# NDLOHGRP/pyReCoDe

Measured on AMD Instinct MI355X. Metric: frames/sec + GB/s in, 4096x4096 uint16 @1% sparsity, 1/2/4/8 GPU, higher is better.
Workload: dtype u16; 1 GPU; 4096x4096 uint16, 1.00% sparsity, L1 + LZ4 frame, source_bit_depth 16, batch 64 frames/GPU/step, 256-frame stack/GPU in HBM; parallelism=dp1 (contiguous frame blocks per rank; single process: no collective), gather_every=0, gathers_issued_in_all=0, launch=single process, collective_ranks=1

## Files before the change

### pyrecode_amd/csrc/rc_api.hip

```cpp
#include "rc_host.h"

thread_local std::string g_last_error;
WorkerPool *g_pool = new WorkerPool;
Util g_utils[RC_MAX_DEV];
thread_local Util *t_util = nullptr;


struct rc_ctx {
    int device = 0;
    hipStream_t own_stream = nullptr, stream = nullptr;
    uint32_t nx = 0, ny = 0, depth = 0, level = 0, op_mode = 0, scheme = 0, clevel = 0, max_batch = 0;
    uint32_t emit = rc::EMIT_RAW;
    rc::Scratch sc, sets[2];
    int cur = 0;
    int last = 0;
    hipStream_t pstream = nullptr;
    hipStream_t pstream_b = nullptr;
    hipStream_t last_ps = nullptr;
    bool two_chains = false;
    hipEvent_t ev_red[2] = {}, ev_post[2] = {}, ev_in[2] = {};
    bool post_pending[2] = {false, false};
    bool pipelined = false;
    bool thr_set = false;
    bool keep_bitmap = true;
    uint32_t src_bytes = 2;
    uint32_t *thr32 = nullptr;
    uint32_t last_n = 0;
    uint8_t *d_frames = nullptr;  uint64_t d_frames_cap = 0;
    uint8_t *d_out = nullptr;     uint64_t d_out_cap = 0;
    uint8_t *d_dark = nullptr;    uint64_t d_dark_cap = 0;
    uint64_t *d_rec_off = nullptr;
    uint32_t *d_md = nullptr;
    void *d_ztab = nullptr;
    bool modelled = false, model_ready = false;
    rc::ZstdModel *d_model = nullptr, *h_model = nullptr;
    rc::ZstdSample *d_sample = nullptr, *h_sample = nullptr;
    uint32_t l2_sum = 0;
    rc::u32x2 *d_l2_node[2] = {};
    uint16_t *d_l2_base[2] = {};
    rc::BatchStatus *h_status = nullptr;
    rc::BatchStatus *d_first_err = nullptr;
    uint32_t batch_seq = 0;
    const uint8_t *prev_out = nullptr, *prev_rec = nullptr, *prev_md = nullptr;
    uint64_t prev_out_cap = 0;
    uint32_t prev_n = 0;
    hipEvent_t ev[5] = {};
// ... 87 lines not shown
        sc.pixraw_stride = ((sc.N * 2 + 15) & ~15ull) + 32;
        sc.nchunk_max = (uint32_t)((sc.N * 2 + PIX_CHUNK - 1) / PIX_CHUNK) + 1;
        HIP_TRY(hipMalloc((void **)&sc.pixraw, B * sc.pixraw_stride + 64));
        HIP_TRY(hipMalloc((void **)&sc.pix_chunks, B * (uint64_t)sc.nchunk_max * PIX_SLOT + 64));
        HIP_TRY(hipMalloc((void **)&sc.chunk_size, B * (uint64_t)sc.nchunk_max * 4));
        HIP_TRY(hipMalloc((void **)&sc.chunk_off, B * (uint64_t)sc.nchunk_max * 4));
        HIP_TRY(hipMalloc((void **)&sc.frame_pbytes, B * 4));
        HIP_TRY(hipMemset(sc.frame_pbytes, 0, B * 4));
    }
    HIP_TRY(hipMemset(sc.frame_nnz, 0, B * 4));
    HIP_TRY(hipMemset(sc.frame_cbytes, 0, B * 4));
    HIP_TRY(hipMemset(sc.status, 0, sizeof(BatchStatus)));
    return RC_OK;
}

static int ctx_alloc(rc_ctx *c)
{
    using namespace rc;
    const uint64_t B = c->max_batch;
    RC_ON_DEVICE(c->device);
    HIP_TRY(hipStreamCreateWithFlags(&c->own_stream, hipStreamNonBlocking));
    HIP_TRY(hipStreamCreateWithFlags(&c->pstream, hipStreamNonBlocking));
    {
        int lo = 0, hi = 0;
        HIP_TRY(hipDeviceGetStreamPriorityRange(&lo, &hi));
        HIP_TRY(hipStreamCreateWithPriority(&c->pstream_b, hipStreamNonBlocking, hi));
    }
    c->last_ps = c->pstream;
    c->stream = c->own_stream;
    HIP_TRY(hipMalloc((void **)&c->sc.thr, c->sc.N * 2));
    HIP_TRY(hipMalloc((void **)&c->d_first_err, sizeof(BatchStatus)));
    HIP_TRY(hipMemset(c->d_first_err, 0, sizeof(BatchStatus)));
    c->sc.first_err = c->d_first_err;
    for (Scratch &set : c->sets) {
        set = c->sc;
        int r = alloc_set(c, set);
        if (r != RC_OK) return r;
    }
    c->two_chains = false;
    if (c->level == 2) {
        const uint64_t ids = (uint64_t)c->sc.ntiles * rc::TILE_PX;
        HIP_TRY(hipMalloc((void **)&c->d_l2_node[0], B * ids * 8));
        HIP_TRY(hipMemset(c->d_l2_node[0], 0, B * ids * 8));
        HIP_TRY(hipMalloc((void **)&c->d_l2_base[0], B * (uint64_t)c->sc.ntiles * 64 * 2));
        for (int i = 0; i < 2; ++i) {
            Scratch &set = c->sets[i];
            set.l2_node = c->d_l2_node[0]; set.l2_ids_per_frame = ids; set.l2_base = c->d_l2_base[0];
        }
    }
    c->sc = c->sets[0];
    if (c->emit == EMIT_ZSTD) {
        std::vector<uint8_t> tab(zstd_tables_bytes());
        zstd_tables_host(tab.data());
        HIP_TRY(hipMalloc(&c->d_ztab, tab.size()));
        HIP_TRY(hipMemcpy(c->d_ztab, tab.data(), tab.size(), hipMemcpyHostToDevice));
        c->modelled = c->clevel != 0;
        if (c->modelled) {
            HIP_TRY(hipMalloc((void **)&c->d_model, sizeof(ZstdModel)));
            HIP_TRY(hipMalloc((void **)&c->d_sample, sizeof(ZstdSample)));
            HIP_TRY(hipHostMalloc((void **)&c->h_model, sizeof(ZstdModel), hipHostMallocDefault));
            HIP_TRY(hipHostMalloc((void **)&c->h_sample, sizeof(ZstdSample), hipHostMallocDefault));
        }
    }
    HIP_TRY(hipMalloc((void **)&c->d_rec_off, (B + 1) * 8));
    HIP_TRY(hipMalloc((void **)&c->d_md, B * 3 * 4));
    HIP_TRY(hipHostMalloc((void **)&c->h_status, 2 * sizeof(BatchStatus), hipHostMallocDefault));
// ... 27 lines not shown
        *status = fail(RC_ERR_UNSUPPORTED, "reduction_level 4 (centroiding) is not implemented on device");
        return nullptr;
    }
    if (reduction_level == 2 && nx > 65535u) {
        *status = fail(RC_ERR_UNSUPPORTED, "reduction_level 2 needs nx <= 65535");
        return nullptr;
    }
    if (src_bit_depth < 1 || src_bit_depth > 32) {
        *status = fail(RC_ERR_UNSUPPORTED, "source_bit_depth must be 1..32 (uint8 / uint16 / uint32 source frames)");
        return nullptr;
    }
    int ndev = 0;
    if (hipGetDeviceCount(&ndev) != hipSuccess || device_id < 0 || device_id >= ndev) {
        (void)hipGetLastError();
        *status = fail(RC_ERR_DEVICE, "no such HIP device (this library has no CPU path)");
        return nullptr;
    }
    rc_ctx *c = new (std::nothrow) rc_ctx();
    if (!c) {
        *status = fail(RC_ERR_DEVICE, "out of host memory");
        return nullptr;
    }
    c->device = device_id;
    c->nx = nx; c->ny = ny; c->depth = src_bit_depth; c->level = reduction_level; c->op_mode = op_mode;
    c->scheme = scheme; c->clevel = clevel; c->max_batch = max_batch;
    c->emit = (op_mode == 1 && rc_scheme_on_device(scheme)) ? scheme : rc::EMIT_RAW;
    rc::Scratch &sc = c->sc;
    sc.N = (uint64_t)nx * ny;
    sc.ntiles = (uint32_t)((sc.N + rc::TILE_PX - 1) / rc::TILE_PX);
    sc.nb = (sc.N + 7) / 8;
    sc.nb_stride = (uint64_t)sc.ntiles * rc::TILE_BM;
    sc.max_batch = max_batch;
    sc.guarded_loads = getenv("RC_REDUCE_GUARDED_LOADS") != nullptr;
    int rcode = ctx_alloc(c);
    if (rcode != RC_OK) {
        *status = rcode;
        std::string keep = g_last_error;
        rc_ctx_destroy(c);
        g_last_error = keep;
        return nullptr;
    }
    return c;
}

RC_EXPORT int rc_ctx_destroy(rc_ctx *c)
{
    if (!c) return RC_OK;
    DeviceGuard dev_guard_;
    (void)dev_guard_.enter(c->device);
    if (c->stream) (void)hipStreamSynchronize(c->stream);
    if (c->pstream) (void)hipStreamSynchronize(c->pstream);
    if (c->pstream_b) (void)hipStreamSynchronize(c->pstream_b);
    if (c->own_stream) (void)hipStreamSynchronize(c->own_stream);
    for (rc::Scratch &sc : c->sets) {
        void *per_set[] = {sc.bitmap, sc.pix_slots, sc.tile_cnt, sc.tile_off, sc.tile_next, sc.blk_slots, sc.blk_size, sc.blk_aux, sc.zl_acc,
                           sc.blk_off, sc.frame_nnz, sc.frame_cbytes, sc.scan_part, sc.status, sc.pixraw, sc.pix_chunks, sc.chunk_size, 
                           sc.chunk_off, sc.frame_pbytes};
        for (void *b : per_set)
            if (b) (void)hipFree(b);
    }
    for (auto &p : c->pipe) {
        void *dev[] = {p.d_in, p.d_out, p.d_rec, p.d_md, p.d_val};
        for (void *b : dev) if (b) (void)hipFree(b);
        void *host[] = {p.h_rec, p.h_md, p.h_stat, p.h_val};
        for (void *b : host) if (b) (void)hipHostFree(b);
        hipEvent_t evs[] = {p.ev_h2d, p.ev_done, p.ev_fetch, p.ev_val};
        for (hipEvent_t e : evs) if (e) (void)hipEventDestroy(e);
    }
    if (c->copy_stream) { (void)hipStreamSynchronize(c->copy_stream); (void)hipStreamDestroy(c->copy_stream); }
    if (c->d2h_stream) { (void)hipStreamSynchronize(c->d2h_stream); (void)hipStreamDestroy(c->d2h_stream); }
    if (c->h_model) (void)hipHostFree(c->h_model);
    if (c->h_sample) (void)hipHostFree(c->h_sample);
    void *bufs[] = {c->sc.thr, c->thr32, c->d_first_err, c->d_frames, c->d_out, c->d_dark, c->d_rec_off,
                    c->d_md, c->d_ztab, c->d_model, c->d_sample, c->d_l2_node[0], c->d_l2_node[1], c->d_l2_base[0], c->d_l2_base[1]};
    for (void *b : bufs)
        if (b) (void)hipFree(b);
    hipEvent_t sync_ev[] = {c->ev_red[0], c->ev_red[1], c->ev_post[0], c->ev_post[1], c->ev_in[0], c->ev_in[1]};
    for (hipEvent_t e : sync_ev)
        if (e) (void)hipEventDestroy(e);
    if (c->pstream) (void)hipStreamDestroy(c->pstream);
    if (c->pstream_b) (void)hipStreamDestroy(c->pstream_b);
    if (c->h_status) (void)hipHostFree(c->h_status);
    for (auto &e : c->ev)
        if (e) (void)hipEventDestroy(e);
    for (auto &e : c->prof_ev) (void)hipEventDestroy(e);
    if (c->own_stream) (void)hipStreamDestroy(c->own_stream);
    delete c;
    return RC_OK;
}

RC_EXPORT int rc_ctx_set_stream(rc_ctx *c, void *hip_stream)
{
    if (!c) return fail(RC_ERR_BAD_ARG, "ctx is NULL");
    c->stream = hip_stream ? reinterpret_cast<hipStream_t>(hip_stream) : c->own_stream;
    return RC_OK;
}

RC_EXPORT int rc_set_threshold(rc_ctx *c, const void *thr)
{
    if (!c || !thr) return fail(RC_ERR_BAD_ARG, "ctx / thr is NULL");
    if (c->depth > 16 && c->src_bytes != 4) return fail(RC_ERR_BAD_ARG, "src_bit_depth > 16 means uint32 sources: rc_ctx_set_source_bytes(ctx, 4) first");
    RC_ON_DEVICE(c->device);
    HIP_TRY(hipMemcpyAsync(c->src_bytes == 4 ? (void *)c->thr32 : (void *)c->sc.thr, thr, c->sc.N * (c->src_bytes == 4 ? 4 : 2),
                           is_device_ptr(thr) ? hipMemcpyDeviceToDevice : hipMemcpyHostToDevice,
                           c->stream));
    HIP_TRY(hipStreamSynchronize(c->stream));
// ... 710 lines not shown
```

### pyrecode_amd/csrc/rc_launch.h

```cpp
#pragma once
#include <hip/hip_runtime.h>
#include <stdint.h>

#include "../../include/recode_hip.h"
#include "rc_device.h"

namespace rc {

constexpr uint32_t COMB_OFF = 0u;
constexpr uint32_t COMB_BEHIND_BLOCK = 1u;
constexpr uint32_t COMB_AT_BLK_SLOT = 2u;

struct Scratch {
    uint64_t N = 0;
    uint32_t ntiles = 0;
    uint64_t nb = 0;
    uint64_t nb_stride = 0;
    uint32_t max_batch = 0;
    bool guarded_loads = false;
    uint16_t *thr = nullptr;
    uint8_t *bitmap = nullptr;
    uint16_t *pix_slots = nullptr;
    uint32_t pix_slot_bytes = SLOT_PX * 2;
    uint32_t *tile_cnt = nullptr;
    uint32_t *tile_off = nullptr;
    uint32_t *tile_next = nullptr;
    uint8_t *blk_slots = nullptr;
    uint32_t blk_stride = BLK_SLOT;
    uint32_t comb = COMB_OFF;
    uint32_t *blk_size = nullptr;
    uint32_t *blk_aux = nullptr;
    uint32_t *zl_acc = nullptr;
    uint32_t *blk_off = nullptr;
    uint32_t *frame_nnz = nullptr;
    uint32_t *frame_cbytes = nullptr;
    uint32_t *scan_part = nullptr;
    BatchStatus *status = nullptr;
    BatchStatus *first_err = nullptr;
    uint8_t *pixraw = nullptr;
    uint64_t pixraw_stride = 0;
    uint8_t *pix_chunks = nullptr;
    uint32_t *chunk_size = nullptr;
    uint32_t *chunk_off = nullptr;
    uint32_t *frame_pbytes = nullptr;
    uint32_t nchunk_max = 0;
    const void *zm_model = nullptr;
    const void *zm_lit_code = nullptr;
    uint32_t zm_valid = 0, zm_budget = 0, zm_seq_bits = 12;
    u32x2 *l2_node = nullptr;
    uint64_t l2_ids_per_frame = 0;
    uint16_t *l2_base = nullptr;
};

// ... 86 lines not shown
```

### pyrecode_amd/csrc/rc_reduce.hip

```cpp
#include <cstddef>
#include <cstdlib>
#include <type_traits>

#include "rc_launch.h"
#include "rc_record.h"
#include "rc_pack.h"
#ifdef RC_PHASE_TIMING
__device__ unsigned long long g_phase[16];
#define RC_LZ4_PHASE 1
#endif
#include "rc_lz4_block.h"
#include "rc_zstd_wave.h"
#include "rc_deflate_block.h"

namespace rc {

#ifdef RC_PHASE_TIMING
#define RC_PHASE_BEGIN unsigned long long ph_t_ = __builtin_amdgcn_s_memtime(); unsigned long long ph_a_[8] = {};
#define RC_PHASE(i) do { const unsigned long long ph_n_ = __builtin_amdgcn_s_memtime(); ph_a_[i] = ph_n_ - ph_t_; ph_t_ = ph_n_; \
        if ((i) == 6 && lane_id() == 0 && (blockIdx.x & 63u) == 0) { for (int q_ = 0; q_ < 7; ++q_) atomicAdd(&g_phase[q_], ph_a_[q_]); atomicAdd(&g_phase[7], 1ull); } } while (0)
#else
#define RC_PHASE_BEGIN
#define RC_PHASE(i) do { } while (0)
#endif
constexpr int REDUCE_BZ = 4;

__device__ __forceinline__ uint32_t pk_sub_sat_u16(uint32_t a, uint32_t b)
{
    uint32_t r;
    asm("v_pk_sub_u16 %0, %1, %2 clamp" : "=v"(r) : "v"(a), "v"(b));
    return r;
}
__device__ __forceinline__ uint32_t pk_add_u16(uint32_t a, uint32_t b)
{
    uint32_t r;
    asm("v_pk_add_u16 %0, %1, %2" : "=v"(r) : "v"(a), "v"(b));
    return r;
}
__device__ __forceinline__ uint32_t pk_min_u16(uint32_t a, uint32_t b)
{
    uint32_t r;
    asm("v_pk_min_u16 %0, %1, %2" : "=v"(r) : "v"(a), "v"(b));
    return r;
}

__global__ void k_threshold(const uint16_t *__restrict__ dark, uint32_t eps16, uint64_t N, uint16_t *__restrict__ thr)
{
    uint64_t i = (uint64_t)blockIdx.x * blockDim.x + threadIdx.x;
    const uint64_t stride = (uint64_t)gridDim.x * blockDim.x;
    for (; i < N; i += stride) thr[i] = (uint16_t)(dark[i] + eps16);
}

__global__ void k_threshold8(const uint8_t *__restrict__ dark, uint32_t eps8, uint64_t N, uint16_t *__restrict__ thr)
{
    uint64_t i = (uint64_t)blockIdx.x * blockDim.x + threadIdx.x;
    const uint64_t stride = (uint64_t)gridDim.x * blockDim.x;
// ... 98 lines not shown
    default: asm volatile("global_load_dwordx4 %0, %1, off offset:3072 nt" : "=&v"(xr) : "v"(p) : "memory"); break;
    }
}
__device__ __forceinline__ void vm_issue_load1(u32x2 &xr, const uint8_t *p, int r)
{
    switch (r) {
    case 0: asm volatile("global_load_dwordx2 %0, %1, off nt" : "=&v"(xr) : "v"(p) : "memory"); break;
    case 1: asm volatile("global_load_dwordx2 %0, %1, off offset:512 nt" : "=&v"(xr) : "v"(p) : "memory"); break;
    case 2: asm volatile("global_load_dwordx2 %0, %1, off offset:1024 nt" : "=&v"(xr) : "v"(p) : "memory"); break;
    case 3: asm volatile("global_load_dwordx2 %0, %1, off offset:1536 nt" : "=&v"(xr) : "v"(p) : "memory"); break;
    case 4: asm volatile("global_load_dwordx2 %0, %1, off offset:2048 nt" : "=&v"(xr) : "v"(p) : "memory"); break;
    case 5: asm volatile("global_load_dwordx2 %0, %1, off offset:2560 nt" : "=&v"(xr) : "v"(p) : "memory"); break;
    case 6: asm volatile("global_load_dwordx2 %0, %1, off offset:3072 nt" : "=&v"(xr) : "v"(p) : "memory"); break;
    default: asm volatile("global_load_dwordx2 %0, %1, off offset:3584 nt" : "=&v"(xr) : "v"(p) : "memory"); break;
    }
}
template <class X>
__device__ __forceinline__ void vm_wait_loads(uint32_t later, X (&x)[R])
{
    switch (later) {
    case 1: asm volatile("s_waitcnt vmcnt(1)" ::: "memory"); break;
    case 2: asm volatile("s_waitcnt vmcnt(2)" ::: "memory"); break;
    case 3: asm volatile("s_waitcnt vmcnt(3)" ::: "memory"); break;
    case 4: asm volatile("s_waitcnt vmcnt(4)" ::: "memory"); break;
    case 5: asm volatile("s_waitcnt vmcnt(5)" ::: "memory"); break;
    case 6: asm volatile("s_waitcnt vmcnt(6)" ::: "memory"); break;
    case 7: asm volatile("s_waitcnt vmcnt(7)" ::: "memory"); break;
    case 8: asm volatile("s_waitcnt vmcnt(8)" ::: "memory"); break;
    default: asm volatile("s_waitcnt vmcnt(0)" ::: "memory"); break;
    }
    asm volatile("" : "+v"(x[0]), "+v"(x[1]), "+v"(x[2]), "+v"(x[3]), "+v"(x[4]), "+v"(x[5]), "+v"(x[6]), "+v"(x[7]) :: "memory");
}

constexpr int STAGE_CAP = 256;
struct __attribute__((aligned(16))) WaveStage {
    uint16_t val[TILE_PX];
    uint16_t out[STAGE_CAP];
};
static_assert(offsetof(WaveStage, out) == sizeof(uint16_t) * TILE_PX && STAGE_CAP >= 64, "compact_dense_in_place: `out` lies right behind `val`, an entry per lane");

__device__ __forceinline__ uint32_t store_lines2(const uint8_t *s0, uint8_t *d0, uint32_t q0, const uint8_t *s1, uint8_t *d1, uint32_t q1)
{
    const uint32_t total = q0 + q1, lane = (uint32_t)lane_id();
    for (uint32_t base = 0; base < total; base += 64) {
        const uint32_t i = base + lane;
        if (i < total) {
            const bool second = i >= q0;
            const uint32_t j = second ? i - q0 : i;
            const u32x4 v = *reinterpret_cast<const u32x4 *>((second ? s1 : s0) + 16 * j);
            *reinterpret_cast<u32x4 *>((second ? d1 : d0) + 16 * j) = v;
        }
    }
    return (total + 63u) >> 6;
}

template <bool LEVEL1, int CODEC, bool KEEP_BITMAP>
__device__ __forceinline__ uint32_t flush_pending(const Pending &p, uint32_t tile, uint32_t n_blk, uint8_t *__restrict__ bitmap,
                                                  uint64_t nb_stride, uint16_t *__restrict__ pix_slots, uint32_t *__restrict__ tile_cnt,
                                                  uint8_t *__restrict__ blk_slots, uint32_t *__restrict__ blk_size, Lz4Lds *lz,
                                                  const WaveStage *st, uint32_t blk_stride, uint32_t comb, uint32_t *__restrict__ blk_aux)
{
    if (!p.valid) return 0;
    const int lane = lane_id();
    uint32_t nst = 0;
    const uint8_t *s0 = nullptr, *s1 = nullptr;
    uint8_t *d0 = nullptr, *d1 = nullptr;
// ... 84 lines not shown
{
    const int lane = lane_id();
    uint32_t *out32 = reinterpret_cast<uint32_t *>(st->out);
    *reinterpret_cast<u32x2 *>(out32 + 2 * lane) = u32x2{0u, 0u};
    __builtin_amdgcn_wave_barrier();
    const uint16_t *mine = st->val + 64 * lane;
    uint64_t q = (uint64_t)own[0] | ((uint64_t)own[1] << 32);
    uint32_t left = cnt, P = 12u * exc;
    do {
        uint32_t x[4];
#pragma unroll
        for (int k = 0; k < 4; ++k) {
            const uint32_t i = q ? (uint32_t)__builtin_ctzll(q) : 0u;
            q &= q - 1;
            x[k] = mine[i];
        }
#pragma unroll
        for (int k = 0; k < 4; ++k) x[k] = (uint32_t)k < left ? (x[k] & 0xFFFu) : 0u;
        const uint32_t lo = x[0] | (x[1] << 12) | (x[2] << 24), hi = (x[2] >> 8) | (x[3] << 4);
        const uint32_t w = P >> 5, sh = P & 31u;
        const uint64_t a = (uint64_t)lo << sh, b = (uint64_t)hi << sh;
        const uint32_t d0 = (uint32_t)a, d1 = (uint32_t)(a >> 32) | (uint32_t)b, d2 = (uint32_t)(b >> 32);
        if (left) {
            __hip_atomic_fetch_or(&out32[w], d0, __ATOMIC_RELAXED, __HIP_MEMORY_SCOPE_WAVEFRONT);
            if (d1) __hip_atomic_fetch_or(&out32[w + 1], d1, __ATOMIC_RELAXED, __HIP_MEMORY_SCOPE_WAVEFRONT);
            if (d2) __hip_atomic_fetch_or(&out32[w + 2], d2, __ATOMIC_RELAXED, __HIP_MEMORY_SCOPE_WAVEFRONT);
        }
        left = left > 4u ? left - 4u : 0u;
        P += 48u;
    } while (__builtin_amdgcn_ballot_w64(left != 0) != 0);
    __builtin_amdgcn_wave_barrier();
}

template <bool ALIGNED, bool ASMLOAD, bool LEVEL1, int CODEC, bool KEEP_BITMAP, bool RAWVAL, int SB>
__device__ __forceinline__ void reduce_one_frame(typename Src<SB>::X (&x)[R], const typename Src<SB>::T *__restrict__ cur, const typename Src<SB>::T *__restrict__ next, bool have_next,
                                                 const u32x4 (&t)[R], uint64_t lane_px0, uint64_t N, bool full,
                                                 uint32_t f, uint32_t tile, uint64_t ft, uint32_t n_blk, uint8_t *__restrict__ bitmap,
                                                 uint64_t nb_stride, uint16_t *__restrict__ pix_slots,
                                                 uint32_t *__restrict__ tile_cnt, uint8_t *__restrict__ blk_slots,
                                                 uint32_t *__restrict__ blk_size, Lz4Lds *s_lz, uint8_t *s_bm, WaveStage *st,
                                                 Pending &pend, uint32_t &stores_behind, const ZmParams &zp, uint32_t blk_stride, uint32_t comb,
                                                 uint32_t *__restrict__ blk_aux)
{
    const int lane = lane_id();
    RC_PHASE_BEGIN
    if (ASMLOAD) vm_wait_loads(stores_behind, x);
    else if (ALIGNED && full) {
        typedef typename Src<SB>::X XU __attribute__((aligned(SB)));
        const XU *p = reinterpret_cast<const XU *>(cur + lane_px0);
#pragma unroll
        for (int r = 0; r < R; ++r) x[r] = __builtin_nontemporal_load(p + r * (GROUP_PX / 8));
    } else {
#pragma unroll
        for (int r = 0; r < R; ++r) x[r] = load8<ALIGNED, true, SB>(cur, lane_px0 + (uint64_t)r * GROUP_PX, N, 0);
    }
    RC_PHASE(0);
    uint32_t m8[R];
#pragma unroll
    for (int r = 0; r < R; ++r) {
        const u32x4 tt = t[r];
        u32x4 xv = widen8(x[r]);
#pragma unroll
        for (int k = 0; k < 4; ++k) xv[k] = pk_sub_sat_u16(xv[k], tt[k]);
        const uint32_t one = 0x00010001u;
        uint32_t M = 0;
#pragma unroll
        for (int k = 3; k >= 0; --k)
            M = __builtin_amdgcn_udot2(__builtin_bit_cast(u16x2, pk_min_u16(xv[k], one)),
                                       __builtin_bit_cast(u16x2, (uint32_t)((1u << (2 * k)) | (2u << (2 * k + 16)))), M, false);
        m8[r] = M;
        if (LEVEL1) {
            u32x4 v = xv;
            if (RAWVAL) {
#pragma unroll
                for (int k = 0; k < 4; ++k) v[k] = pk_add_u16(v[k], tt[k]);
            }
            (reinterpret_cast<u32x4 *>(st->val) + lane)[r * 64] = v;
        }
        if (ASMLOAD && have_next) vm_issue_load1(x[r], next + lane_px0, r);
    }
    RC_PHASE(1);
    RC_PHASE(2);
    pend.valid = true;
    pend.ft = ft;
    pend.f = f;
    pend.cnt = 0;
    pend.csize = 0;
    pend.buf = st->out;
    if (LEVEL1 || KEEP_BITMAP || CODEC) {
        uint8_t *bm = CODEC ? s_lz->raw : s_bm;
#pragma unroll
        for (int r = 0; r < R; ++r) bm[r * 64 + lane] = (uint8_t)m8[r];
        __builtin_amdgcn_wave_barrier();
        pend.own = *reinterpret_cast<const u32x2 *>(&bm[lane * 8]);
    }
    RC_PHASE(3);
    if (LEVEL1) {
        const uint32_t cnt = (uint32_t)__builtin_popcount(pend.own[0]) + (uint32_t)__builtin_popcount(pend.own[1]);
        const uint32_t inc = wave_incl_scan(cnt);
        const uint32_t wave_total = wave_last(inc);
        bool packed = false;
        if (pend.depth == 12 && wave_total <= FUSED12_CAP) {
            if (wave_total) compact_pack12(st, pend.own, inc - cnt, cnt);
            packed = true;
        } else if (wave_total <= (uint32_t)STAGE_CAP) {
#pragma unroll
            for (int h = 0; h < 2; ++h) {
                const uint16_t *mine = st->val + 64 * lane + 32 * h;
                uint32_t qh = pend.own[h];
                uint32_t o = inc - cnt + (h ? (uint32_t)__builtin_popcount(pend.own[0]) : 0u);
                while (qh) {
                    const uint32_t i0 = (uint32_t)__builtin_ctz(qh);
// ... 19 lines not shown
    RC_PHASE(4);
    if (CODEC == CODEC_LZ4_RUNS) {
        const uint64_t bytes = (uint64_t)pend.own[0] | ((uint64_t)pend.own[1] << 32);
        pend.csize = lz4_encode_block<false>(bytes, n_blk, *s_lz);
    }
    if (CODEC == CODEC_LZ4_EVENTS) {
        const uint64_t bytes = (uint64_t)pend.own[0] | ((uint64_t)pend.own[1] << 32);
        pend.csize = lz4_encode_block<true>(bytes, n_blk, *s_lz);
    }
    if (CODEC == CODEC_ZSTD_FAST) {
        const uint64_t bytes = (uint64_t)pend.own[0] | ((uint64_t)pend.own[1] << 32);
        pend.csize = zstd_tokenize_block(bytes, n_blk, pend.last, *s_lz, pend.staged);
    }
    if (CODEC == CODEC_ZSTD_MODELLED) {
        const uint64_t bytes = (uint64_t)pend.own[0] | ((uint64_t)pend.own[1] << 32);
        pend.csize = zstd_tokenize_block_m(bytes, n_blk, pend.last, *s_lz, pend.staged, zp);
    }
    if (CODEC == CODEC_DEFLATE) {
        const uint64_t bytes = (uint64_t)pend.own[0] | ((uint64_t)pend.own[1] << 32);
        pend.aux = deflate_adler_word(bytes, tile);
        pend.csize = deflate_encode_block<true>(bytes, n_blk, pend.last, *s_lz);
    }
    if (CODEC == CODEC_BLOSC) {
        const uint64_t bytes = (uint64_t)pend.own[0] | ((uint64_t)pend.own[1] << 32);
        pend.cown = bitshuffle_block(bytes, n_blk, *s_lz);
        pend.csize = lz4_encode_block(pend.cown, n_blk, *s_lz);
    }
    RC_PHASE(5);
    stores_behind = flush_pending<LEVEL1, CODEC, KEEP_BITMAP>(pend, tile, n_blk, bitmap, nb_stride, pix_slots, tile_cnt, blk_slots, blk_size, s_lz, st, blk_stride, comb, blk_aux);
    pend.valid = false;
    RC_PHASE(6);
}

template <int RWAVES, int BZ, bool ALIGNED, bool ASMLOAD, bool LEVEL1, int CODEC, bool KEEP_BITMAP, bool RAWVAL, int SB>
__global__ __launch_bounds__(64 * RWAVES) __attribute__((amdgpu_waves_per_eu((ALIGNED && ASMLOAD) ? ((RWAVES == 4 && LEVEL1) ? 3 : 4) : 1))) void k_reduce_tiles(const typename Src<SB>::T *__restrict__ frames,
                                                       const uint16_t *__restrict__ thr, uint64_t N, uint32_t ntiles,
                                                       uint32_t tile0, uint32_t tile_end,
                                                       uint32_t B, uint32_t ngroups, uint64_t nb,
                                                       uint8_t *__restrict__ bitmap, uint64_t nb_stride,
                                                       uint16_t *__restrict__ pix_slots, uint32_t *__restrict__ tile_cnt,
                                                       uint8_t *__restrict__ blk_slots, uint32_t *__restrict__ blk_size, uint32_t depth,
                                                       BatchStatus *__restrict__ status, ZmParams zm, uint32_t blk_stride, uint32_t comb,
                                                       uint32_t *__restrict__ blk_aux)
{
    if (blockIdx.x == 0 && threadIdx.x == 0) { status->code = 0; status->frame = 0; status->total = 0; }
    __shared__ uint16_t s_code[CODEC == CODEC_ZSTD_MODELLED ? 256 : 2];
    if (CODEC == CODEC_ZSTD_MODELLED) {
        for (uint32_t i = threadIdx.x; i < 128; i += 64 * RWAVES) reinterpret_cast<uint32_t *>(s_code)[i] = reinterpret_cast<const uint32_t *>(zm.lit_code)[i];
        __syncthreads();
        zm.lit_code = s_code;
    }
    __shared__ Lz4Lds s_lz[CODEC ? RWAVES : 1];
    __shared__ __attribute__((aligned(16))) uint8_t s_bm[CODEC ? 1 : RWAVES][CODEC ? 16 : TILE_BM];
    __shared__ WaveStage s_stage[LEVEL1 ? RWAVES : 1];

    const uint32_t xcd = blockIdx.x & 7u, j = blockIdx.x >> 3;
    const uint32_t grp = j % ngroups;
    const uint32_t tblock = (j / ngroups) * 8u + xcd;
    const int lane = lane_id();
    const int w = __builtin_amdgcn_readfirstlane((int)(threadIdx.x >> 6));
    const uint32_t tile = tile0 + tblock * RWAVES + w;
    if (tile >= tile_end) return;
    const uint64_t lane_px0 = (uint64_t)tile * TILE_PX + (uint64_t)lane * 8;
    const uint32_t f0 = grp * BZ;
    if (f0 >= B) return;
    const bool full = (uint64_t)(tile + 1) * TILE_PX <= N;

    typename Src<SB>::X xa[R];
    if (ASMLOAD) vm_issue_loads(xa, frames + (uint64_t)f0 * N + lane_px0);
    u32x4 t[R];
#pragma unroll
    for (int r = 0; r < R; ++r) t[r] = load8<ALIGNED, false, 2>(thr, lane_px0 + (uint64_t)r * GROUP_PX, N, 0xFFFF);
    const uint32_t n_blk = (uint32_t)min((uint64_t)TILE_BM, nb - (uint64_t)tile * TILE_BM);
    Lz4Lds *lz = &s_lz[CODEC ? w : 0];
    uint8_t *bm = s_bm[CODEC ? 0 : w];
    WaveStage *st = &s_stage[LEVEL1 ? w : 0];
    Pending pend;
    pend.valid = false;
    pend.ft = 0; pend.f = 0; pend.cnt = 0; pend.csize = 0; pend.own = u32x2{0u, 0u};
    pend.staged = 0; pend.last = tile + 1 == ntiles; pend.cown = 0; pend.aux = 0;
    pend.depth = (LEVEL1 && !RAWVAL) ? depth : 16u;
    pend.buf = nullptr;

    uint32_t stores_behind = 0;
#pragma unroll 1
    for (int z = 0; z < BZ; ++z) {
        const uint32_t f = f0 + z;
        if (f >= B) break;
        const bool nxt = z + 1 < BZ && f + 1 < B;
        reduce_one_frame<ALIGNED, ASMLOAD, LEVEL1, CODEC, KEEP_BITMAP, RAWVAL, SB>(xa, frames + (uint64_t)f * N, frames + (uint64_t)(f + 1) * N, nxt, t,
                                                                             lane_px0, N, full, f, tile, (uint64_t)f * ntiles + tile, n_blk,
                                                                             bitmap, nb_stride, pix_slots, tile_cnt, blk_slots,
                                                                             blk_size, lz, bm, st, pend, stores_behind, zm, blk_stride, comb, blk_aux);
        if (!nxt) break;
    }
    flush_pending<LEVEL1, CODEC, KEEP_BITMAP>(pend, tile, n_blk, bitmap, nb_stride, pix_slots, tile_cnt, blk_slots, blk_size, lz, st, blk_stride, comb, blk_aux);
}

template <int BZ, bool AL, bool L1, int CODEC, bool KEEP, bool RAW, int SB>
static void launch_reduce_t(const Scratch &sc, const typename Src<SB>::T *frames, uint32_t B, uint32_t depth, hipStream_t s, hipStream_t s_tail)
{
    const uint32_t ngroups = (B + BZ - 1) / BZ;
    const uint32_t nfull = AL ? (uint32_t)(sc.N / TILE_PX) : 0u;
    const ZmParams zm{reinterpret_cast<const uint16_t *>(sc.zm_lit_code), sc.zm_valid, sc.zm_budget, sc.zm_seq_bits};
    const uint32_t comb = (L1 && !RAW && CODEC) ? sc.comb : COMB_OFF;
    const bool three = L1 && !RAW && CODEC != CODEC_DEFLATE &&
                       (CODEC == CODEC_LZ4_RUNS || CODEC == CODEC_LZ4_EVENTS || sc.ntiles > 8192 || (CODEC == CODEC_ZSTD_MODELLED && (sc.zm_valid & ZM_LITS_ONLY)));
    auto go = [&](auto rw) {
        constexpr int RW = decltype(rw)::value;
        auto grid_for = [&](uint32_t nt) { return (((nt + RW - 1) / RW + 7) / 8) * 8 * ngroups; };
        if (nfull)
            hipLaunchKernelGGL((k_reduce_tiles<RW, BZ, AL, AL, L1, CODEC, KEEP, RAW, SB>), dim3(grid_for(nfull)), dim3(64 * RW), 0, s, frames, sc.thr, sc.N,
                               sc.ntiles, 0u, nfull, B, ngroups, sc.nb, sc.bitmap, sc.nb_stride, sc.pix_slots, sc.tile_cnt, sc.blk_slots,
                               sc.blk_size, depth, sc.status, zm, sc.blk_stride, comb, sc.blk_aux);
        if (nfull < sc.ntiles) {
            if (AL && sc.N % 8 != 0)
                hipLaunchKernelGGL((k_reduce_tiles<RW, BZ, false, false, L1, CODEC, KEEP, RAW, SB>), dim3(grid_for(sc.ntiles - nfull)), dim3(64 * RW), 0, nfull ? s_tail : s, frames,
                                   sc.thr, sc.N, sc.ntiles, nfull, sc.ntiles, B, ngroups, sc.nb, sc.bitmap, sc.nb_stride, sc.pix_slots, sc.tile_cnt,
                                   sc.blk_slots, sc.blk_size, depth, sc.status, zm, sc.blk_stride, comb, sc.blk_aux);
            else
                hipLaunchKernelGGL((k_reduce_tiles<RW, BZ, AL, false, L1, CODEC, KEEP, RAW, SB>), dim3(grid_for(sc.ntiles - nfull)), dim3(64 * RW), 0, nfull ? s_tail : s, frames,
                                   sc.thr, sc.N, sc.ntiles, nfull, sc.ntiles, B, ngroups, sc.nb, sc.bitmap, sc.nb_stride, sc.pix_slots, sc.tile_cnt,
                                   sc.blk_slots, sc.blk_size, depth, sc.status, zm, sc.blk_stride, comb, sc.blk_aux);
        }
    };
    if constexpr (SB == 2) {
        if (three) { go(int_c<3>{}); return; }
    }
    go(int_c<4>{});
}
template <int BZ, bool AL, bool L1, bool RAW, int SB>
static void launch_reduce_c(const Scratch &sc, const typename Src<SB>::T *frames, uint32_t B, uint32_t codec, bool keep, uint32_t depth, hipStream_t s, hipStream_t s_tail)
{
    if (RAW) keep = true;
#define RC_CODEC(C)                                                                                      \
    if (codec == C) {                                                                                    \
        if (keep) launch_reduce_t<BZ, AL, L1, C, true, RAW, SB>(sc, frames, B, depth, s, s_tail);        \
        else if (!RAW) launch_reduce_t<BZ, AL, L1, C, false, false, SB>(sc, frames, B, depth, s, s_tail); \
        return;                                                                                          \
    }
    RC_CODEC(CODEC_LZ4_RUNS) RC_CODEC(CODEC_LZ4_EVENTS) RC_CODEC(CODEC_ZSTD_FAST) RC_CODEC(CODEC_ZSTD_MODELLED) RC_CODEC(CODEC_BLOSC) RC_CODEC(CODEC_DEFLATE)
#undef RC_CODEC
    launch_reduce_t<BZ, AL, L1, CODEC_NONE, true, RAW, SB>(sc, frames, B, depth, s, s_tail);
}
template <int BZ, bool AL, int SB>
static void launch_reduce_a(const Scratch &sc, const typename Src<SB>::T *frames, uint32_t B, uint32_t level, uint32_t codec, bool keep,
                            uint32_t depth, hipStream_t s, hipStream_t s_tail)
{
    if (level == 2) launch_reduce_c<BZ, AL, true, true, SB>(sc, frames, B, codec, keep, depth, s, s_tail);
    else if (level == 1) launch_reduce_c<BZ, AL, true, false, SB>(sc, frames, B, codec, keep, depth, s, s_tail);
    else launch_reduce_c<BZ, AL, false, false, SB>(sc, frames, B, codec, keep, depth, s, s_tail);
}
#ifdef RC_PHASE_TIMING
extern "C" __attribute__((visibility("default"))) int rc_debug_phases(unsigned long long *out16)
{
    unsigned long long z[16] = {};
    if (hipDeviceSynchronize() != hipSuccess) return -1;
    if (hipMemcpyFromSymbol(out16, HIP_SYMBOL(g_phase), sizeof z) != hipSuccess) return -1;
    if (hipMemcpyToSymbol(HIP_SYMBOL(g_phase), z, sizeof z) != hipSuccess) return -1;
    return 0;
// ... 450 lines not shown
```

Baseline: 156,800 frames/s.

## Replace static tile grid with persistent waves pulling work items via atomic counters

For the three-wave aligned uint16 reduce path, the launch now starts a persistent grid sized to resident workgroups (CUs × 5). Each wave pulls (tile, frame-group) items from per-XCD atomic counters, with monotonic bases so the counters need no reset between launches. The next item's frame and threshold loads are prefetched with nontemporal inline-asm loads while the current item is processed. The goal is to remove tail imbalance and launch overhead of a grid that is ngroups times larger. In exchange it adds atomic traffic, pins v127 as a reserved register with a 127-VGPR cap, and depends on host-side counter bookkeeping staying in sync with the device.

Result: slower. 133,700 frames/s (-14.8%).

```diff
diff --git a/pyrecode_amd/csrc/rc_api.hip b/pyrecode_amd/csrc/rc_api.hip
--- a/pyrecode_amd/csrc/rc_api.hip
+++ b/pyrecode_amd/csrc/rc_api.hip
@@ -12,6 +12,8 @@
     uint32_t nx = 0, ny = 0, depth = 0, level = 0, op_mode = 0, scheme = 0, clevel = 0, max_batch = 0;
     uint32_t emit = rc::EMIT_RAW;
     rc::Scratch sc, sets[2];
+    rc::ItemPull items;
+    uint32_t item_start = 0;
     int cur = 0;
     int last = 0;
     hipStream_t pstream = nullptr;
@@ -165,6 +167,18 @@
     HIP_TRY(hipMalloc((void **)&c->d_first_err, sizeof(BatchStatus)));
     HIP_TRY(hipMemset(c->d_first_err, 0, sizeof(BatchStatus)));
     c->sc.first_err = c->d_first_err;
+    {
+        hipDeviceProp_t prop;
+        HIP_TRY(hipGetDeviceProperties(&prop, c->device));
+        c->items.resident_wgs = (uint32_t)prop.multiProcessorCount * 5u;
+        if (const char *e = getenv("RC_EXP_ITEM_WGS")) c->items.resident_wgs = (uint32_t)atoi(e);
+        c->items.sum_groups = 0;
+        c->items.sum_waves = c->item_start;
+        const std::vector<uint32_t> init(8 * ITEM_CTR_STRIDE, c->item_start);
+        HIP_TRY(hipMalloc((void **)&c->items.ctr, init.size() * 4));
+        HIP_TRY(hipMemcpy(c->items.ctr, init.data(), init.size() * 4, hipMemcpyHostToDevice));
+        c->sc.items = &c->items;
+    }
     for (Scratch &set : c->sets) {
         set = c->sc;
         int r = alloc_set(c, set);
@@ -258,6 +272,7 @@
     sc.nb_stride = (uint64_t)sc.ntiles * rc::TILE_BM;
     sc.max_batch = max_batch;
     sc.guarded_loads = getenv("RC_REDUCE_GUARDED_LOADS") != nullptr;
+    if (const char *e = getenv("RC_REDUCE_ITEM_START")) c->item_start = (uint32_t)strtoul(e, nullptr, 0);
     int rcode = ctx_alloc(c);
     if (rcode != RC_OK) {
         *status = rcode;
@@ -297,7 +312,7 @@
     if (c->d2h_stream) { (void)hipStreamSynchronize(c->d2h_stream); (void)hipStreamDestroy(c->d2h_stream); }
     if (c->h_model) (void)hipHostFree(c->h_model);
     if (c->h_sample) (void)hipHostFree(c->h_sample);
-    void *bufs[] = {c->sc.thr, c->thr32, c->d_first_err, c->d_frames, c->d_out, c->d_dark, c->d_rec_off,
+    void *bufs[] = {c->sc.thr, c->thr32, c->d_first_err, c->items.ctr, c->d_frames, c->d_out, c->d_dark, c->d_rec_off,
                     c->d_md, c->d_ztab, c->d_model, c->d_sample, c->d_l2_node[0], c->d_l2_node[1], c->d_l2_base[0], c->d_l2_base[1]};
     for (void *b : bufs)
         if (b) (void)hipFree(b);
diff --git a/pyrecode_amd/csrc/rc_launch.h b/pyrecode_amd/csrc/rc_launch.h
--- a/pyrecode_amd/csrc/rc_launch.h
+++ b/pyrecode_amd/csrc/rc_launch.h
@@ -11,6 +11,14 @@
 constexpr uint32_t COMB_BEHIND_BLOCK = 1u;
 constexpr uint32_t COMB_AT_BLK_SLOT = 2u;
 
+constexpr uint32_t ITEM_CTR_STRIDE = 32;
+struct ItemPull {
+    uint32_t *ctr = nullptr;
+    uint32_t sum_groups = 0;
+    uint32_t sum_waves = 0;
+    uint32_t resident_wgs = 0;
+};
+
 struct Scratch {
     uint64_t N = 0;
     uint32_t ntiles = 0;
@@ -19,6 +27,7 @@
     uint32_t max_batch = 0;
     bool guarded_loads = false;
     uint16_t *thr = nullptr;
+    ItemPull *items = nullptr;
     uint8_t *bitmap = nullptr;
     uint16_t *pix_slots = nullptr;
     uint32_t pix_slot_bytes = SLOT_PX * 2;
diff --git a/pyrecode_amd/csrc/rc_reduce.hip b/pyrecode_amd/csrc/rc_reduce.hip
--- a/pyrecode_amd/csrc/rc_reduce.hip
+++ b/pyrecode_amd/csrc/rc_reduce.hip
@@ -1,5 +1,6 @@
 #include <cstddef>
 #include <cstdlib>
+#include <tuple>
 #include <type_traits>
 
 #include "rc_launch.h"
@@ -19,9 +20,11 @@
 #define RC_PHASE_BEGIN unsigned long long ph_t_ = __builtin_amdgcn_s_memtime(); unsigned long long ph_a_[8] = {};
 #define RC_PHASE(i) do { const unsigned long long ph_n_ = __builtin_amdgcn_s_memtime(); ph_a_[i] = ph_n_ - ph_t_; ph_t_ = ph_n_; \
         if ((i) == 6 && lane_id() == 0 && (blockIdx.x & 63u) == 0) { for (int q_ = 0; q_ < 7; ++q_) atomicAdd(&g_phase[q_], ph_a_[q_]); atomicAdd(&g_phase[7], 1ull); } } while (0)
+#define RC_PHASE_FIRST(first) do { if ((first) && lane_id() == 0 && (blockIdx.x & 63u) == 0) { atomicAdd(&g_phase[14], ph_a_[0]); atomicAdd(&g_phase[15], 1ull); } } while (0)
 #else
 #define RC_PHASE_BEGIN
 #define RC_PHASE(i) do { } while (0)
+#define RC_PHASE_FIRST(first) do { } while (0)
 #endif
 constexpr int REDUCE_BZ = 4;
 
@@ -186,6 +189,68 @@
     asm volatile("" : "+v"(x[0]), "+v"(x[1]), "+v"(x[2]), "+v"(x[3]), "+v"(x[4]), "+v"(x[5]), "+v"(x[6]), "+v"(x[7]) :: "memory");
 }
 
+struct LaneOff { uint32_t lo, hi; };
+template <bool NT>
+__device__ __forceinline__ void vm_issue_group(u32x4 &xr, const uint16_t *tile_base, const LaneOff &lo, int r)
+{
+    const uint32_t v = r >= 4 ? lo.hi : lo.lo;
+    if (NT) {
+        switch (r & 3) {
+        case 0: asm volatile("global_load_dwordx4 %0, %1, %2 nt" : "=&v"(xr) : "v"(v), "s"(tile_base) : "memory"); break;
+        case 1: asm volatile("global_load_dwordx4 %0, %1, %2 offset:1024 nt" : "=&v"(xr) : "v"(v), "s"(tile_base) : "memory"); break;
+        case 2: asm volatile("global_load_dwordx4 %0, %1, %2 offset:2048 nt" : "=&v"(xr) : "v"(v), "s"(tile_base) : "memory"); break;
+        default: asm volatile("global_load_dwordx4 %0, %1, %2 offset:3072 nt" : "=&v"(xr) : "v"(v), "s"(tile_base) : "memory"); break;
+        }
+    } else {
+        switch (r & 3) {
+        case 0: asm volatile("global_load_dwordx4 %0, %1, %2" : "=&v"(xr) : "v"(v), "s"(tile_base) : "memory"); break;
+        case 1: asm volatile("global_load_dwordx4 %0, %1, %2 offset:1024" : "=&v"(xr) : "v"(v), "s"(tile_base) : "memory"); break;
+        case 2: asm volatile("global_load_dwordx4 %0, %1, %2 offset:2048" : "=&v"(xr) : "v"(v), "s"(tile_base) : "memory"); break;
+        default: asm volatile("global_load_dwordx4 %0, %1, %2 offset:3072" : "=&v"(xr) : "v"(v), "s"(tile_base) : "memory"); break;
+        }
+    }
+}
+__device__ __forceinline__ void vm_issue_pull(uint32_t *ctr)
+{
+    uint64_t saved;
+    const uint32_t one = 1u;
+    asm volatile("s_mov_b64 %0, exec\n\t"
+                 "s_mov_b64 exec, 1\n\t"
+                 "global_atomic_add v127, %1, %2, off sc0\n\t"
+                 "s_mov_b64 exec, %0"
+                 : "=&s"(saved) : "v"(ctr), "v"(one) : "memory", "v127");
+}
+template <bool WAIT_ALL>
+__device__ __forceinline__ uint32_t vm_take_pull()
+{
+    uint32_t r;
+    if (WAIT_ALL) asm volatile("s_waitcnt vmcnt(0)\n\tv_readfirstlane_b32 %0, v127" : "=s"(r) :: "memory");
+    else asm volatile("v_readfirstlane_b32 %0, v127" : "=s"(r) :: "memory");
+    return r;
+}
+__device__ __forceinline__ void vm_fence_thr(u32x4 (&t)[R])
+{
+    asm volatile("" : "+v"(t[0]), "+v"(t[1]), "+v"(t[2]), "+v"(t[3]), "+v"(t[4]), "+v"(t[5]), "+v"(t[6]), "+v"(t[7]) :: "memory");
+}
+struct ItemLists {
+    uint32_t ntl, ngroups, sum_groups, sum_waves;
+    __device__ __forceinline__ uint32_t tiles(uint32_t l) const { return (ntl + 7u - l) >> 3; }
+    __device__ __forceinline__ uint32_t len(uint32_t l) const { return tiles(l) * ngroups; }
+    __device__ __forceinline__ uint32_t base(uint32_t l) const { return tiles(l) * sum_groups + sum_waves; }
+};
+constexpr uint32_t NO_ITEM = 0xFFFFFFFFu;
+__device__ __forceinline__ uint32_t pull_now(uint32_t *ctr, const ItemLists &il, uint32_t xcd, uint32_t &k)
+{
+    while (k < 8u) {
+        const uint32_t l = (xcd + k) & 7u;
+        vm_issue_pull(ctr + l * ITEM_CTR_STRIDE);
+        const uint32_t idx = vm_take_pull<true>() - il.base(l);
+        if (idx < il.len(l)) return idx;
+        ++k;
+    }
+    return NO_ITEM;
+}
+
 constexpr int STAGE_CAP = 256;
 struct __attribute__((aligned(16))) WaveStage {
     uint16_t val[TILE_PX];
@@ -336,9 +401,9 @@
     __builtin_amdgcn_wave_barrier();
 }
 
-template <bool ALIGNED, bool ASMLOAD, bool LEVEL1, int CODEC, bool KEEP_BITMAP, bool RAWVAL, int SB>
-__device__ __forceinline__ void reduce_one_frame(typename Src<SB>::X (&x)[R], const typename Src<SB>::T *__restrict__ cur, const typename Src<SB>::T *__restrict__ next, bool have_next,
-                                                 const u32x4 (&t)[R], uint64_t lane_px0, uint64_t N, bool full,
+template <bool ALIGNED, bool ASMLOAD, bool LEVEL1, int CODEC, bool KEEP_BITMAP, bool RAWVAL, int SB, bool PULL, class Hook>
+__device__ __forceinline__ void reduce_one_frame(typename Src<SB>::X (&x)[R], const typename Src<SB>::T *__restrict__ cur, const typename Src<SB>::T *next, bool have_next,
+                                                 u32x4 (&t)[R], Hook &&after_wait, const LaneOff &off, bool item_first, uint64_t lane_px0, uint64_t N, bool full,
                                                  uint32_t f, uint32_t tile, uint64_t ft, uint32_t n_blk, uint8_t *__restrict__ bitmap,
                                                  uint64_t nb_stride, uint16_t *__restrict__ pix_slots,
                                                  uint32_t *__restrict__ tile_cnt, uint8_t *__restrict__ blk_slots,
@@ -348,8 +413,11 @@
 {
     const int lane = lane_id();
     RC_PHASE_BEGIN
-    if (ASMLOAD) vm_wait_loads(stores_behind, x);
-    else if (ALIGNED && full) {
+    const uint16_t *thr_next = nullptr;
+    if (ASMLOAD) {
+        vm_wait_loads(stores_behind, x);
+        if (PULL) { vm_fence_thr(t); after_wait(next, have_next, thr_next); }
+    } else if (ALIGNED && full) {
         typedef typename Src<SB>::X XU __attribute__((aligned(SB)));
         const XU *p = reinterpret_cast<const XU *>(cur + lane_px0);
 #pragma unroll
@@ -359,6 +427,7 @@
         for (int r = 0; r < R; ++r) x[r] = load8<ALIGNED, true, SB>(cur, lane_px0 + (uint64_t)r * GROUP_PX, N, 0);
     }
     RC_PHASE(0);
+    RC_PHASE_FIRST(item_first);
     uint32_t m8[R];
 #pragma unroll
     for (int r = 0; r < R; ++r) {
@@ -381,7 +450,12 @@
             }
             (reinterpret_cast<u32x4 *>(st->val) + lane)[r * 64] = v;
         }
-        if (ASMLOAD && have_next) vm_issue_load1(x[r], next + lane_px0, r);
+        if (ASMLOAD && have_next) {
+            if constexpr (PULL && SB == 2) {
+                vm_issue_group<true>(x[r], next, off, r);
+                if (thr_next) vm_issue_group<false>(t[r], thr_next, off, r);
+            } else vm_issue_load1(x[r], next, r);
+        }
     }
     RC_PHASE(1);
     RC_PHASE(2);
@@ -467,8 +541,8 @@
     RC_PHASE(6);
 }
 
-template <int RWAVES, int BZ, bool ALIGNED, bool ASMLOAD, bool LEVEL1, int CODEC, bool KEEP_BITMAP, bool RAWVAL, int SB>
-__global__ __launch_bounds__(64 * RWAVES) __attribute__((amdgpu_waves_per_eu((ALIGNED && ASMLOAD) ? ((RWAVES == 4 && LEVEL1) ? 3 : 4) : 1))) void k_reduce_tiles(const typename Src<SB>::T *__restrict__ frames,
+template <int RWAVES, int BZ, bool ALIGNED, bool ASMLOAD, bool LEVEL1, int CODEC, bool KEEP_BITMAP, bool RAWVAL, int SB, bool PULL>
+__device__ __forceinline__ void reduce_tiles_body(const typename Src<SB>::T *__restrict__ frames,
                                                        const uint16_t *__restrict__ thr, uint64_t N, uint32_t ntiles,
                                                        uint32_t tile0, uint32_t tile_end,
                                                        uint32_t B, uint32_t ngroups, uint64_t nb,
@@ -476,8 +550,9 @@
                                                        uint16_t *__restrict__ pix_slots, uint32_t *__restrict__ tile_cnt,
                                                        uint8_t *__restrict__ blk_slots, uint32_t *__restrict__ blk_size, uint32_t depth,
                                                        BatchStatus *__restrict__ status, ZmParams zm, uint32_t blk_stride, uint32_t comb,
-                                                       uint32_t *__restrict__ blk_aux)
-{
+                                                       uint32_t *__restrict__ blk_aux, uint32_t *item_ctr, uint32_t item_sum_groups, uint32_t item_sum_waves)
+{
+    static_assert(!PULL || (ALIGNED && ASMLOAD && SB == 2), "items are pulled by the steady-state instantiation only");
     if (blockIdx.x == 0 && threadIdx.x == 0) { status->code = 0; status->frame = 0; status->total = 0; }
     __shared__ uint16_t s_code[CODEC == CODEC_ZSTD_MODELLED ? 256 : 2];
     if (CODEC == CODEC_ZSTD_MODELLED) {
@@ -489,6 +564,65 @@
     __shared__ __attribute__((aligned(16))) uint8_t s_bm[CODEC ? 1 : RWAVES][CODEC ? 16 : TILE_BM];
     __shared__ WaveStage s_stage[LEVEL1 ? RWAVES : 1];
 
+    if constexpr (PULL) {
+        const int lane = lane_id();
+        const int w = __builtin_amdgcn_readfirstlane((int)(threadIdx.x >> 6));
+        const uint32_t xcd = blockIdx.x & 7u;
+        const ItemLists il{tile_end, ngroups, item_sum_groups, item_sum_waves};
+        uint32_t k = 0;
+        uint32_t idx = pull_now(item_ctr, il, xcd, k);
+        if (idx == NO_ITEM) return;
+        uint32_t tile = (idx / ngroups) * 8u + ((xcd + k) & 7u), f0 = (idx % ngroups) * BZ;
+        const LaneOff off{(uint32_t)lane * 16u, (uint32_t)lane * 16u + 4096u};
+        typename Src<SB>::X xa[R];
+        u32x4 t[R];
+#pragma unroll
+        for (int r = 0; r < R; ++r) vm_issue_group<true>(xa[r], frames + (uint64_t)f0 * N + (uint64_t)tile * TILE_PX, off, r);
+#pragma unroll
+        for (int r = 0; r < R; ++r) vm_issue_group<false>(t[r], thr + (uint64_t)tile * TILE_PX, off, r);
+        Lz4Lds *lz = &s_lz[CODEC ? w : 0];
+        uint8_t *bm = s_bm[CODEC ? 0 : w];
+        WaveStage *st = &s_stage[LEVEL1 ? w : 0];
+        Pending pend;
+        pend.valid = false;
+        pend.ft = 0; pend.f = 0; pend.cnt = 0; pend.csize = 0; pend.own = u32x2{0u, 0u};
+        pend.staged = 0; pend.last = false; pend.cown = 0; pend.aux = 0;
+        pend.depth = (LEVEL1 && !RAWVAL) ? depth : 16u;
+        pend.buf = nullptr;
+        uint32_t stores_behind = 0;
+#pragma unroll 1
+        for (;;) {
+            const uint32_t nz = min((uint32_t)BZ, B - f0);
+            const uint32_t n_blk = (uint32_t)min((uint64_t)TILE_BM, nb - (uint64_t)tile * TILE_BM);
+            pend.last = tile + 1 == ntiles;
+            uint32_t ntile = 0, nf0 = 0;
+            bool succ = false;
+#pragma unroll 1
+            for (uint32_t z = 0; z < nz; ++z) {
+                const uint32_t f = f0 + z;
+                const bool last = z + 1 == nz;
+                auto after_wait = [&](const typename Src<SB>::T *&next, bool &have_next, const uint16_t *&thr_next) {
+                    if (z + 2 == nz || nz == 1u) vm_issue_pull(item_ctr + ((xcd + k) & 7u) * ITEM_CTR_STRIDE);
+                    if (!last) return;
+                    uint32_t nidx = (nz == 1u ? vm_take_pull<true>() : vm_take_pull<false>()) - il.base((xcd + k) & 7u);
+                    if (nidx >= il.len((xcd + k) & 7u)) { ++k; nidx = pull_now(item_ctr, il, xcd, k); }
+                    if (nidx == NO_ITEM) return;
+                    succ = true;
+                    ntile = (nidx / ngroups) * 8u + ((xcd + k) & 7u);
+                    nf0 = (nidx % ngroups) * BZ;
+                    have_next = true;
+                    next = frames + (uint64_t)nf0 * N + (uint64_t)ntile * TILE_PX;
+                    if (ntile != tile) thr_next = thr + (uint64_t)ntile * TILE_PX;
+                };
+                reduce_one_frame<ALIGNED, ASMLOAD, LEVEL1, CODEC, KEEP_BITMAP, RAWVAL, SB, true>(xa, frames + (uint64_t)f * N, frames + (uint64_t)(f + 1) * N + (uint64_t)tile * TILE_PX, !last, t, after_wait, off, z == 0,
+                                                                                       0, N, true, f, tile, (uint64_t)f * ntiles + tile, n_blk,
+                                                                                       bitmap, nb_stride, pix_slots, tile_cnt, blk_slots,
+                                                                                       blk_size, lz, bm, st, pend, stores_behind, zm, blk_stride, comb, blk_aux);
+            }
+            if (!succ) return;
+            tile = ntile; f0 = nf0;
+        }
+    } else {
     const uint32_t xcd = blockIdx.x & 7u, j = blockIdx.x >> 3;
     const uint32_t grp = j % ngroups;
     const uint32_t tblock = (j / ngroups) * 8u + xcd;
@@ -506,6 +640,7 @@
     u32x4 t[R];
 #pragma unroll
     for (int r = 0; r < R; ++r) t[r] = load8<ALIGNED, false, 2>(thr, lane_px0 + (uint64_t)r * GROUP_PX, N, 0xFFFF);
+    auto no_hook = [](const typename Src<SB>::T *&, bool &, const uint16_t *&) {};
     const uint32_t n_blk = (uint32_t)min((uint64_t)TILE_BM, nb - (uint64_t)tile * TILE_BM);
     Lz4Lds *lz = &s_lz[CODEC ? w : 0];
     uint8_t *bm = s_bm[CODEC ? 0 : w];
@@ -523,13 +658,50 @@
         const uint32_t f = f0 + z;
         if (f >= B) break;
         const bool nxt = z + 1 < BZ && f + 1 < B;
-        reduce_one_frame<ALIGNED, ASMLOAD, LEVEL1, CODEC, KEEP_BITMAP, RAWVAL, SB>(xa, frames + (uint64_t)f * N, frames + (uint64_t)(f + 1) * N, nxt, t,
+        reduce_one_frame<ALIGNED, ASMLOAD, LEVEL1, CODEC, KEEP_BITMAP, RAWVAL, SB, false>(xa, frames + (uint64_t)f * N, frames + (uint64_t)(f + 1) * N + lane_px0, nxt, t, no_hook, LaneOff{0u, 0u}, z == 0,
                                                                              lane_px0, N, full, f, tile, (uint64_t)f * ntiles + tile, n_blk,
                                                                              bitmap, nb_stride, pix_slots, tile_cnt, blk_slots,
                                                                              blk_size, lz, bm, st, pend, stores_behind, zm, blk_stride, comb, blk_aux);
         if (!nxt) break;
     }
     flush_pending<LEVEL1, CODEC, KEEP_BITMAP>(pend, tile, n_blk, bitmap, nb_stride, pix_slots, tile_cnt, blk_slots, blk_size, lz, st, blk_stride, comb, blk_aux);
+    }
+}
+
+#define RC_REDUCE_WAVES_PER_EU amdgpu_waves_per_eu((ALIGNED && ASMLOAD) ? ((RWAVES == 4 && LEVEL1) ? 3 : 4) : 1)
+template <int RWAVES, int BZ, bool ALIGNED, bool ASMLOAD, bool LEVEL1, int CODEC, bool KEEP_BITMAP, bool RAWVAL, int SB, bool PULL = false, std::enable_if_t<!PULL, int> = 0>
+__global__ __launch_bounds__(64 * RWAVES) __attribute__((RC_REDUCE_WAVES_PER_EU)) void k_reduce_tiles(const typename Src<SB>::T *__restrict__ frames,
+                                                       const uint16_t *__restrict__ thr, uint64_t N, uint32_t ntiles,
+                                                       uint32_t tile0, uint32_t tile_end,
+                                                       uint32_t B, uint32_t ngroups, uint64_t nb,
+                                                       uint8_t *__restrict__ bitmap, uint64_t nb_stride,
+                                                       uint16_t *__restrict__ pix_slots, uint32_t *__restrict__ tile_cnt,
+                                                       uint8_t *__restrict__ blk_slots, uint32_t *__restrict__ blk_size, uint32_t depth,
+                                                       BatchStatus *__restrict__ status, ZmParams zm, uint32_t blk_stride, uint32_t comb,
+                                                       uint32_t *__restrict__ blk_aux, uint32_t *item_ctr, uint32_t item_sum_groups, uint32_t item_sum_waves)
+{
+    reduce_tiles_body<RWAVES, BZ, ALIGNED, ASMLOAD, LEVEL1, CODEC, KEEP_BITMAP, RAWVAL, SB, false>(frames, thr, N, ntiles, tile0, tile_end, B, ngroups, nb, bitmap, nb_stride, pix_slots, tile_cnt, blk_slots, blk_size, depth, status, zm, blk_stride, comb, blk_aux, item_ctr, item_sum_groups, item_sum_waves);
+}
+template <int RWAVES, int BZ, bool ALIGNED, bool ASMLOAD, bool LEVEL1, int CODEC, bool KEEP_BITMAP, bool RAWVAL, int SB, bool PULL, std::enable_if_t<PULL, int> = 0>
+__global__ __launch_bounds__(64 * RWAVES) __attribute__((amdgpu_num_vgpr(127))) __attribute__((RC_REDUCE_WAVES_PER_EU)) void k_reduce_tiles(const typename Src<SB>::T *__restrict__ frames,
+                                                       const uint16_t *__restrict__ thr, uint64_t N, uint32_t ntiles,
+                                                       uint32_t tile0, uint32_t tile_end,
+                                                       uint32_t B, uint32_t ngroups, uint64_t nb,
+                                                       uint8_t *__restrict__ bitmap, uint64_t nb_stride,
+                                                       uint16_t *__restrict__ pix_slots, uint32_t *__restrict__ tile_cnt,
+                                                       uint8_t *__restrict__ blk_slots, uint32_t *__restrict__ blk_size, uint32_t depth,
+                                                       BatchStatus *__restrict__ status, ZmParams zm, uint32_t blk_stride, uint32_t comb,
+                                                       uint32_t *__restrict__ blk_aux, uint32_t *item_ctr, uint32_t item_sum_groups, uint32_t item_sum_waves)
+{
+    reduce_tiles_body<RWAVES, BZ, ALIGNED, ASMLOAD, LEVEL1, CODEC, KEEP_BITMAP, RAWVAL, SB, true>(frames, thr, N, ntiles, tile0, tile_end, B, ngroups, nb, bitmap, nb_stride, pix_slots, tile_cnt, blk_slots, blk_size, depth, status, zm, blk_stride, comb, blk_aux, item_ctr, item_sum_groups, item_sum_waves);
+}
+#undef RC_REDUCE_WAVES_PER_EU
+
+template <class... P, class... A>
+static hipError_t launch_status(void (*kern)(P...), dim3 grid, dim3 block, hipStream_t s, A... a)
+{
+    std::tuple<std::remove_cv_t<P>...> v(static_cast<P>(a)...);
+    return std::apply([&](auto &...e) { void *p[] = {static_cast<void *>(&e)...}; return hipLaunchKernel(reinterpret_cast<const void *>(kern), grid, block, p, 0, s); }, v);
 }
 
 template <int BZ, bool AL, bool L1, int CODEC, bool KEEP, bool RAW, int SB>
@@ -544,23 +716,33 @@
     auto go = [&](auto rw) {
         constexpr int RW = decltype(rw)::value;
         auto grid_for = [&](uint32_t nt) { return (((nt + RW - 1) / RW + 7) / 8) * 8 * ngroups; };
-        if (nfull)
+        if constexpr (RW == 3 && AL && SB == 2) {
+            if (nfull) {
+                ItemPull &ip = *sc.items;
+                const uint64_t nitems = (uint64_t)nfull * ngroups;
+                const uint32_t grid = (uint32_t)std::min<uint64_t>(ip.resident_wgs, (nitems + RW - 1) / RW);
+                const hipError_t e = launch_status(k_reduce_tiles<RW, BZ, AL, AL, L1, CODEC, KEEP, RAW, SB, true>, dim3(grid), dim3(64 * RW), s, frames, sc.thr, sc.N,
+                                                   sc.ntiles, 0u, nfull, B, ngroups, sc.nb, sc.bitmap, sc.nb_stride, sc.pix_slots, sc.tile_cnt, sc.blk_slots,
+                                                   sc.blk_size, depth, sc.status, zm, sc.blk_stride, comb, sc.blk_aux, ip.ctr, ip.sum_groups, ip.sum_waves);
+                if (e == hipSuccess) { ip.sum_groups += ngroups; ip.sum_waves += grid * RW; }
+            }
+        } else if (nfull)
             hipLaunchKernelGGL((k_reduce_tiles<RW, BZ, AL, AL, L1, CODEC, KEEP, RAW, SB>), dim3(grid_for(nfull)), dim3(64 * RW), 0, s, frames, sc.thr, sc.N,
                                sc.ntiles, 0u, nfull, B, ngroups, sc.nb, sc.bitmap, sc.nb_stride, sc.pix_slots, sc.tile_cnt, sc.blk_slots,
-                               sc.blk_size, depth, sc.status, zm, sc.blk_stride, comb, sc.blk_aux);
+                               sc.blk_size, depth, sc.status, zm, sc.blk_stride, comb, sc.blk_aux, nullptr, 0u, 0u);
         if (nfull < sc.ntiles) {
             if (AL && sc.N % 8 != 0)
                 hipLaunchKernelGGL((k_reduce_tiles<RW, BZ, false, false, L1, CODEC, KEEP, RAW, SB>), dim3(grid_for(sc.ntiles - nfull)), dim3(64 * RW), 0, nfull ? s_tail : s, frames,
                                    sc.thr, sc.N, sc.ntiles, nfull, sc.ntiles, B, ngroups, sc.nb, sc.bitmap, sc.nb_stride, sc.pix_slots, sc.tile_cnt,
-                                   sc.blk_slots, sc.blk_size, depth, sc.status, zm, sc.blk_stride, comb, sc.blk_aux);
+                                   sc.blk_slots, sc.blk_size, depth, sc.status, zm, sc.blk_stride, comb, sc.blk_aux, nullptr, 0u, 0u);
             else
                 hipLaunchKernelGGL((k_reduce_tiles<RW, BZ, AL, false, L1, CODEC, KEEP, RAW, SB>), dim3(grid_for(sc.ntiles - nfull)), dim3(64 * RW), 0, nfull ? s_tail : s, frames,
                                    sc.thr, sc.N, sc.ntiles, nfull, sc.ntiles, B, ngroups, sc.nb, sc.bitmap, sc.nb_stride, sc.pix_slots, sc.tile_cnt,
-                                   sc.blk_slots, sc.blk_size, depth, sc.status, zm, sc.blk_stride, comb, sc.blk_aux);
+                                   sc.blk_slots, sc.blk_size, depth, sc.status, zm, sc.blk_stride, comb, sc.blk_aux, nullptr, 0u, 0u);
         }
     };
     if constexpr (SB == 2) {
-        if (three) { go(int_c<3>{}); return; }
+        if (three && sc.items) { go(int_c<3>{}); return; }
     }
     go(int_c<4>{});
 }
```
